# modelscope/FunCodec

Hardware: NVIDIA H100
Metric: codec frames/sec (encode+RVQ+decode) (higher is better)
Workload: dtype f32

## Files before the change

### funcodec_b200/csrc/rvq_tc.cu

```cuda
#include <climits>
#include "common.cuh"
#include "kernels.h"
#include "tc_sm90.cuh"

namespace fcb {

using namespace tc;

constexpr int RQ_M = 128;
constexpr int RQ_N = RVQ_TC_N;
constexpr int RQ_NB = 2;
constexpr int RQ_THREADS = 160;
constexpr float RQ_RESCORE_TOL = 4e-3f;

struct RqSmem {
    int a_slab;
    int off_b, off_cc, off_xx, off_idx, off_cand, off_bar, total;
};

__host__ __device__ inline RqSmem rq_layout(int D, int K) {
    RqSmem L;
    const int n_chunks = D / 32;
    L.a_slab = RQ_M * 128;
    L.off_b = 2 * n_chunks * L.a_slab;
    L.off_cc = L.off_b + RQ_NB * 2 * RQ_N * 128;
    L.off_xx = L.off_cc + K * 4;
    L.off_idx = L.off_xx + RQ_M * 4;
    L.off_cand = L.off_idx + RQ_M * 4;
    L.off_bar = (L.off_cand + 4 * RQ_M * 4 + 15) & ~15;
    L.total = L.off_bar + 8 * (2 * RQ_NB) + 16;
    return L;
}

__global__ void __launch_bounds__(RQ_THREADS, 1) rvq_tc_kernel(const RvqParams p) {
    extern __shared__ __align__(1024) uint8_t smem_raw[];
    const int tid = threadIdx.x, lane = tid & 31, warp = tid >> 5;
    const int D = p.D, K = p.K, T = p.T;
    const int n_chunks = D / 32;
    const int n_nt = K / RQ_N;
    const RqSmem L = rq_layout(D, K);
    const long long M = (long long)p.B * T;
    const long long row0 = (long long)blockIdx.x * RQ_M;

    uint8_t* smA = smem_raw;
    uint8_t* smB = smem_raw + L.off_b;
    float* cc_s = reinterpret_cast<float*>(smem_raw + L.off_cc);
    float* xx_s = reinterpret_cast<float*>(smem_raw + L.off_xx);
    int* idx_s = reinterpret_cast<int*>(smem_raw + L.off_idx);
    float* cv1_s = reinterpret_cast<float*>(smem_raw + L.off_cand);
    float* cv2_s = cv1_s + RQ_M;
    int* ci1_s = reinterpret_cast<int*>(cv2_s + RQ_M);
    int* ci2_s = ci1_s + RQ_M;
    uint64_t* bars = reinterpret_cast<uint64_t*>(smem_raw + L.off_bar);
    uint64_t* b_full = bars;
    uint64_t* b_empty = b_full + RQ_NB;

    if (tid == 0) {
        for (int i = 0; i < RQ_NB; ++i) { mbar_init(b_full + i, 1); mbar_init(b_empty + i, 1); }
        mbar_fence_init();
    }
    __syncthreads();
    const long long slab_bytes = 2LL * RQ_N * 128;

    if (warp < 4) {
        const int jchunk = tid & 7, rsub = tid >> 3;
        for (int ch = 0; ch < n_chunks; ++ch) {
            uint8_t* hi = smA + (2 * ch) * L.a_slab;
            uint8_t* lo = hi + L.a_slab;
            for (int r = rsub; r < RQ_M; r += 16) {
                const long long row = row0 + r;
                float4 v = make_float4(0.f, 0.f, 0.f, 0.f);
                const int d = ch * 32 + jchunk * 4;
                if (row < M) {
                    const int b = (int)(row / T), t = (int)(row - (long long)b * T);
                    v = __ldg(reinterpret_cast<const float4*>(p.in.x + (long long)b * p.in.clip_stride + (long long)(p.in.row_off + t) * D + d));
                    if (p.in.stats) {
                        const float mean = p.in.stats[2 * b], rstd = p.in.stats[2 * b + 1];
                        const float4 g4 = __ldg(reinterpret_cast<const float4*>(p.in.gamma + d));
                        const float4 b4 = __ldg(reinterpret_cast<const float4*>(p.in.beta + d));
                        float a;
                        a = rstd * g4.x; v.x = fmaf(v.x, a, b4.x - a * mean);
                        a = rstd * g4.y; v.y = fmaf(v.y, a, b4.y - a * mean);
                        a = rstd * g4.z; v.z = fmaf(v.z, a, b4.z - a * mean);
                        a = rstd * g4.w; v.w = fmaf(v.w, a, b4.w - a * mean);
                    }
                    if (p.enc_out) *reinterpret_cast<float4*>(p.enc_out + row * D + d) = v;
                }
                float4 h, l;
                split_tf32(v.x, h.x, l.x); split_tf32(v.y, h.y, l.y); split_tf32(v.z, h.z, l.z); split_tf32(v.w, h.w, l.w);
                const uint32_t o = (uint32_t)r * 128u + (uint32_t)((jchunk ^ (r & 7)) << 4);
                *reinterpret_cast<float4*>(hi + o) = h;
                *reinterpret_cast<float4*>(lo + o) = l;
            }
        }
        const int myrow = tid;
        const uint32_t a_base = smem_u32(smA), b_base = smem_u32(smB);
        long long it = 0;
        auto lex_lt = [](float va, int ia, float vb, int ib) { return va < vb || (va == vb && ia < ib); };
        for (int q = 0; q < p.n_q; ++q) {
            const float* E = p.embed + (long long)q * K * D;
            asm volatile("bar.sync 1, 128;" ::: "memory");
            for (int r = rsub; r < RQ_M; r += 16) {
                float s = 0.f;
                for (int d = jchunk; d < D; d += 8) {
                    const uint32_t o = (uint32_t)r * 128u + (uint32_t)((((d & 31) >> 2) ^ (r & 7)) << 4) + (uint32_t)((d & 3) << 2);
                    const uint8_t* hi = smA + (2 * (d >> 5)) * L.a_slab;
                    const float v = *reinterpret_cast<const float*>(hi + o) + *reinterpret_cast<const float*>(hi + L.a_slab + o);
                    s = fmaf(v, v, s);
                }
                s += __shfl_xor_sync(0xffffffffu, s, 1);
                s += __shfl_xor_sync(0xffffffffu, s, 2);
                s += __shfl_xor_sync(0xffffffffu, s, 4);
                if (jchunk == 0) xx_s[r] = s;
            }
            for (int c = tid; c < K; c += 128) cc_s[c] = __ldg(p.cnorm + (long long)q * K + c);
            fence_proxy_async_smem();
            asm volatile("bar.sync 1, 128;" ::: "memory");
            const float xx = xx_s[myrow];
            float xr[4], bv1[4], bv2[4];
            int bi1[4], bi2[4];
#pragma unroll
            for (int k = 0; k < 4; ++k) {
                xr[k] = xx_s[64 * (k >> 1) + 16 * warp + (lane >> 2) + 8 * (k & 1)];
                bv1[k] = 3.402823466e38f; bv2[k] = 3.402823466e38f;
                bi1[k] = INT_MAX; bi2[k] = INT_MAX;
            }
            for (int nt = 0; nt < n_nt; ++nt) {
                float acc0[RQ_N / 2], acc1[RQ_N / 2];
                int prev = -1;
                for (int ch = 0; ch < n_chunks; ++ch, ++it) {
                    const int bs = (int)(it % RQ_NB);
                    mbar_wait(b_full + bs, (uint32_t)((it / RQ_NB) & 1));
                    const uint32_t a_hi0 = a_base + (2 * ch) * L.a_slab, a_lo0 = a_hi0 + L.a_slab;
                    const uint32_t b_hi0 = b_base + bs * (uint32_t)slab_bytes, b_lo0 = b_hi0 + RQ_N * 128;
                    wgmma_fence();
#pragma unroll
                    for (int ks = 0; ks < 4; ++ks) {
                        const uint64_t db_hi = make_desc_k_sw128(b_hi0 + ks * 32), db_lo = make_desc_k_sw128(b_lo0 + ks * 32);
                        const uint32_t accum = (ch | ks) != 0;
                        wgmma_m64n128k8_tf32(acc0, make_desc_k_sw128(a_lo0 + ks * 32), db_hi, accum);
                        wgmma_m64n128k8_tf32(acc0, make_desc_k_sw128(a_hi0 + ks * 32), db_lo, 1);
                        wgmma_m64n128k8_tf32(acc0, make_desc_k_sw128(a_hi0 + ks * 32), db_hi, 1);
                        wgmma_m64n128k8_tf32(acc1, make_desc_k_sw128(a_lo0 + 8192 + ks * 32), db_hi, accum);
                        wgmma_m64n128k8_tf32(acc1, make_desc_k_sw128(a_hi0 + 8192 + ks * 32), db_lo, 1);
                        wgmma_m64n128k8_tf32(acc1, make_desc_k_sw128(a_hi0 + 8192 + ks * 32), db_hi, 1);
                    }
                    wgmma_commit();
                    wgmma_wait<1>();
                    if (prev >= 0 && tid == 0) mbar_arrive(b_empty + prev);
                    prev = bs;
                }
                wgmma_wait<0>();
                reg_fence(acc0);
                reg_fence(acc1);
                if (tid == 0) mbar_arrive(b_empty + prev);
                auto scan = [&](const float (&a)[RQ_N / 2], int h) {
#pragma unroll
                    for (int j = 0; j < RQ_N / 8; ++j)
#pragma unroll
                        for (int e = 0; e < 2; ++e) {
                            const int k = 2 * h + e;
#pragma unroll
                            for (int x = 0; x < 2; ++x) {
                                const int c = nt * RQ_N + 8 * j + 2 * (lane & 3) + x;
                                const float tv = __fadd_rn(__fsub_rn(xr[k], 2.0f * a[4 * j + 2 * e + x]), cc_s[c]);
                                if (tv < bv1[k]) { bv2[k] = bv1[k]; bi2[k] = bi1[k]; bv1[k] = tv; bi1[k] = c; }
                                else if (tv < bv2[k]) { bv2[k] = tv; bi2[k] = c; }
                            }
                        }
                };
                scan(acc0, 0);
                scan(acc1, 1);
            }
#pragma unroll
            for (int k = 0; k < 4; ++k) {
#pragma unroll
                for (int o = 1; o <= 2; o <<= 1) {
                    const float ov1 = __shfl_xor_sync(0xffffffffu, bv1[k], o), ov2 = __shfl_xor_sync(0xffffffffu, bv2[k], o);
                    const int oi1 = __shfl_xor_sync(0xffffffffu, bi1[k], o), oi2 = __shfl_xor_sync(0xffffffffu, bi2[k], o);
                    if (lex_lt(ov1, oi1, bv1[k], bi1[k])) {
                        if (lex_lt(ov2, oi2, bv1[k], bi1[k])) { bv2[k] = ov2; bi2[k] = oi2; }
                        else { bv2[k] = bv1[k]; bi2[k] = bi1[k]; }
                        bv1[k] = ov1; bi1[k] = oi1;
                    } else if (lex_lt(ov1, oi1, bv2[k], bi2[k])) {
                        bv2[k] = ov1; bi2[k] = oi1;
                    }
                }
                if ((lane & 3) == 0) {
                    const int rr = 64 * (k >> 1) + 16 * warp + (lane >> 2) + 8 * (k & 1);
                    cv1_s[rr] = bv1[k]; ci1_s[rr] = bi1[k] == INT_MAX ? 0 : bi1[k];
                    cv2_s[rr] = bv2[k]; ci2_s[rr] = bi2[k] == INT_MAX ? -1 : bi2[k];
                }
            }
            asm volatile("bar.sync 1, 128;" ::: "memory");
            const float v1 = cv1_s[myrow], v2 = cv2_s[myrow];
            const int i1 = ci1_s[myrow], i2 = ci2_s[myrow];
            int best = i1;
            if (row0 + myrow < M && v2 - v1 < RQ_RESCORE_TOL + 2e-5f * fabsf(v1) && i2 >= 0) {
                float d1 = 0.f, d2 = 0.f;
                const float* c1 = E + (long long)i1 * D;
                const float* c2 = E + (long long)i2 * D;
                for (int d = 0; d < D; ++d) {
                    const uint32_t o = (uint32_t)myrow * 128u + (uint32_t)((((d & 31) >> 2) ^ (myrow & 7)) << 4) + (uint32_t)((d & 3) << 2);
                    const uint8_t* hi = smA + (2 * (d >> 5)) * L.a_slab;
                    const float x = *reinterpret_cast<const float*>(hi + o) + *reinterpret_cast<const float*>(hi + L.a_slab + o);
                    d1 = fmaf(x, __ldg(c1 + d), d1);
                    d2 = fmaf(x, __ldg(c2 + d), d2);
                }
                const float t1 = __fadd_rn(__fsub_rn(xx, 2.0f * d1), cc_s[i1]);
                const float t2 = __fadd_rn(__fsub_rn(xx, 2.0f * d2), cc_s[i2]);
                if (t2 < t1 || (t2 == t1 && i2 < i1)) best = i2;
            }
            idx_s[myrow] = best;
            if (row0 + myrow < M) p.codes[(long long)q * M + row0 + myrow] = (long long)best;
            asm volatile("bar.sync 1, 128;" ::: "memory");
            {
                constexpr int MAXCH = 4;
                float4 cv[MAXCH], nv[MAXCH];
                auto load_c = [&](int r, float4 (&dst)[MAXCH]) {
#pragma unroll
                    for (int ch = 0; ch < MAXCH; ++ch) {
                        dst[ch] = make_float4(0.f, 0.f, 0.f, 0.f);
                        if (ch < n_chunks && row0 + r < M)
                            dst[ch] = __ldg(reinterpret_cast<const float4*>(E + (long long)idx_s[r] * D + ch * 32 + jchunk * 4));
                    }
                };
                load_c(rsub, cv);
                for (int r = rsub; r < RQ_M; r += 16) {
                    if (r + 16 < RQ_M) load_c(r + 16, nv);
                    const long long row = row0 + r;
                    if (row < M) {
                        const uint32_t o = (uint32_t)r * 128u + (uint32_t)((jchunk ^ (r & 7)) << 4);
#pragma unroll
                        for (int ch = 0; ch < MAXCH; ++ch) {
                            if (ch < n_chunks) {
                                uint8_t* hi = smA + (2 * ch) * L.a_slab;
                                uint8_t* lo = hi + L.a_slab;
                                const float4 h0 = *reinterpret_cast<const float4*>(hi + o);
                                const float4 l0 = *reinterpret_cast<const float4*>(lo + o);
                                const float4 c4 = cv[ch];
                                float4 x;
                                x.x = (h0.x + l0.x) - c4.x; x.y = (h0.y + l0.y) - c4.y; x.z = (h0.z + l0.z) - c4.z; x.w = (h0.w + l0.w) - c4.w;
                                float4 h, l;
                                split_tf32(x.x, h.x, l.x); split_tf32(x.y, h.y, l.y); split_tf32(x.z, h.z, l.z); split_tf32(x.w, h.w, l.w);
                                *reinterpret_cast<float4*>(hi + o) = h;
                                *reinterpret_cast<float4*>(lo + o) = l;
                                if (p.sub_quants) {
                                    const int b = (int)(row / T), t = (int)(row - (long long)b * T);
                                    const int d = ch * 32 + jchunk * 4;
                                    float* sq = p.sub_quants + (((long long)q * p.B + b) * D + d) * T + t;
                                    sq[0] = c4.x; sq[(long long)T] = c4.y; sq[2LL * T] = c4.z; sq[3LL * T] = c4.w;
                                }
                            }
                        }
                    }
#pragma unroll
                    for (int ch = 0; ch < MAXCH; ++ch) cv[ch] = nv[ch];
                }
            }
        }
    } else if (warp == 4) {
        if (lane == 0) {
            long long it = 0;
            for (int q = 0; q < p.n_q; ++q) {
                const uint8_t* qbase = reinterpret_cast<const uint8_t*>(p.embed_tc) + (long long)q * n_nt * n_chunks * slab_bytes;
                for (int nt = 0; nt < n_nt; ++nt)
                    for (int ch = 0; ch < n_chunks; ++ch, ++it) {
                        const int bs = (int)(it % RQ_NB);
                        mbar_wait_backoff(b_empty + bs, (uint32_t)((it / RQ_NB) & 1) ^ 1, 64);
                        mbar_arrive_expect_tx(b_full + bs, (uint32_t)slab_bytes);
                        bulk_g2s(smB + bs * slab_bytes, qbase + ((long long)nt * n_chunks + ch) * slab_bytes, (uint32_t)slab_bytes, b_full + bs);
                    }
            }
        }
    }
}

bool rvq_tc_supported(int D, int K) {
    return D % 32 == 0 && D >= 32 && D <= 128 && K % RQ_N == 0 && rq_layout(D, K).total <= 225 * 1024;
}

cudaError_t launch_rvq_tc(const RvqParams& p, cudaStream_t st) {
    if (!rvq_tc_supported(p.D, p.K) || !p.embed_tc) return cudaErrorInvalidValue;
    const RqSmem L = rq_layout(p.D, p.K);
    {
        cudaError_t e = ensure_dynamic_smem((const void*)rvq_tc_kernel, 225 * 1024);
        if (e != cudaSuccess) return e;
    }
    const long long M = (long long)p.B * p.T;
    rvq_tc_kernel<<<(unsigned)((M + RQ_M - 1) / RQ_M), RQ_THREADS, L.total, st>>>(p);
    return cudaGetLastError();
}

}
```

### funcodec_b200/csrc/tc_sm90.cuh

```cuda
#pragma once
#include <cuda_runtime.h>
#include <stdint.h>

namespace fcb {
namespace tc {

__device__ __forceinline__ uint32_t smem_u32(const void* p) { return (uint32_t)__cvta_generic_to_shared(p); }

__device__ __forceinline__ void mbar_init(uint64_t* bar, uint32_t count) {
    asm volatile("mbarrier.init.shared::cta.b64 [%0], %1;" ::"r"(smem_u32(bar)), "r"(count) : "memory");
}
__device__ __forceinline__ void mbar_fence_init() { asm volatile("fence.mbarrier_init.release.cluster;" ::: "memory"); }
__device__ __forceinline__ void mbar_arrive(uint64_t* bar) {
    asm volatile("{\n\t.reg .b64 st;\n\tmbarrier.arrive.shared::cta.b64 st, [%0];\n\t}" ::"r"(smem_u32(bar)) : "memory");
}
__device__ __forceinline__ void mbar_arrive_expect_tx(uint64_t* bar, uint32_t bytes) {
    asm volatile("{\n\t.reg .b64 st;\n\tmbarrier.arrive.expect_tx.shared::cta.b64 st, [%0], %1;\n\t}" ::"r"(smem_u32(bar)), "r"(bytes)
                 : "memory");
}
__device__ __forceinline__ void mbar_arrive_if(uint64_t* bar, bool pred) {
    asm volatile("{\n\t.reg .pred p;\n\t.reg .b64 st;\n\tsetp.ne.b32 p, %1, 0;\n\t@p mbarrier.arrive.shared::cta.b64 st, [%0];\n\t}" ::"r"(
                     smem_u32(bar)),
                 "r"((uint32_t)pred)
                 : "memory");
}
__device__ __forceinline__ bool mbar_try_wait(uint64_t* bar, uint32_t parity) {
    uint32_t ok;
    asm volatile(
        "{\n\t.reg .pred p;\n\t"
        "mbarrier.try_wait.parity.shared::cta.b64 p, [%1], %2;\n\t"
        "selp.u32 %0, 1, 0, p;\n\t}"
        : "=r"(ok)
        : "r"(smem_u32(bar)), "r"(parity)
        : "memory");
    return ok != 0;
}
__device__ __forceinline__ void mbar_wait(uint64_t* bar, uint32_t parity) {
    while (!mbar_try_wait(bar, parity)) { }
}
__device__ __forceinline__ void mbar_wait_backoff(uint64_t* bar, uint32_t parity, unsigned ns) {
    while (!mbar_try_wait(bar, parity)) { __nanosleep(ns); }
}

__device__ __forceinline__ void mbar_wait_cluster_backoff(uint64_t* bar, uint32_t parity, unsigned ns) {
    for (;;) {
        uint32_t ok;
        asm volatile(
            "{\n\t.reg .pred p;\n\t"
            "mbarrier.try_wait.parity.acquire.cluster.shared::cta.b64 p, [%1], %2;\n\t"
            "selp.u32 %0, 1, 0, p;\n\t}"
            : "=r"(ok)
            : "r"(smem_u32(bar)), "r"(parity)
            : "memory");
        if (ok) return;
        __nanosleep(ns);
    }
}

__device__ __forceinline__ void fence_proxy_async_smem() { asm volatile("fence.proxy.async.shared::cta;" ::: "memory"); }

__device__ __forceinline__ uint32_t cluster_ctarank() {
    uint32_t r;
    asm volatile("mov.u32 %0, %%cluster_ctarank;" : "=r"(r));
    return r;
}
__device__ __forceinline__ uint32_t mapa_shared(uint32_t smem_addr, uint32_t rank) {
    uint32_t r;
    asm volatile("mapa.shared::cluster.u32 %0, %1, %2;" : "=r"(r) : "r"(smem_addr), "r"(rank));
    return r;
}
__device__ __forceinline__ void mbar_arrive_remote_if(uint32_t remote_bar, bool pred) {
    asm volatile("{\n\t.reg .pred p;\n\tsetp.ne.b32 p, %1, 0;\n\t@p mbarrier.arrive.release.cluster.shared::cluster.b64 _, [%0];\n\t}" ::"r"(
                     remote_bar),
                 "r"((uint32_t)pred)
                 : "memory");
}
__device__ __forceinline__ void bulk_s2peer(uint32_t dst_remote, const void* src_smem, uint32_t bytes, uint32_t bar_remote) {
    asm volatile("cp.async.bulk.shared::cluster.shared::cta.mbarrier::complete_tx::bytes [%0], [%1], %2, [%3];" ::"r"(dst_remote),
                 "r"(smem_u32(src_smem)), "r"(bytes), "r"(bar_remote)
                 : "memory");
}
__device__ __forceinline__ void cluster_sync() {
    asm volatile("barrier.cluster.arrive.release;\n\tbarrier.cluster.wait.acquire;" ::: "memory");
}

__device__ __forceinline__ void bulk_g2s(void* dst_smem, const void* src_gmem, uint32_t bytes, uint64_t* bar) {
    asm volatile("cp.async.bulk.shared::cluster.global.mbarrier::complete_tx::bytes [%0], [%1], %2, [%3];" ::"r"(smem_u32(dst_smem)),
                 "l"(src_gmem), "r"(bytes), "r"(smem_u32(bar))
                 : "memory");
}

__device__ __forceinline__ void tma_load_4d(void* dst_smem, const void* tmap, int c0, int c1, int c2, int c3, uint64_t* bar) {
    asm volatile(
        "cp.async.bulk.tensor.4d.shared::cluster.global.tile.mbarrier::complete_tx::bytes [%0], [%1, {%3, %4, %5, %6}], [%2];" ::"r"(
            smem_u32(dst_smem)),
        "l"(tmap), "r"(smem_u32(bar)), "r"(c0), "r"(c1), "r"(c2), "r"(c3)
        : "memory");
}

__device__ __forceinline__ void tma_load_5d(void* dst_smem, const void* tmap, int c0, int c1, int c2, int c3, int c4, uint64_t* bar) {
    asm volatile(
        "cp.async.bulk.tensor.5d.shared::cluster.global.tile.mbarrier::complete_tx::bytes [%0], [%1, {%3, %4, %5, %6, %7}], [%2];" ::"r"(
            smem_u32(dst_smem)),
        "l"(tmap), "r"(smem_u32(bar)), "r"(c0), "r"(c1), "r"(c2), "r"(c3), "r"(c4)
        : "memory");
}

template <int R>
__device__ __forceinline__ void setmaxnreg_dec() { asm volatile("setmaxnreg.dec.sync.aligned.u32 %0;" ::"n"(R)); }
template <int R>
__device__ __forceinline__ void setmaxnreg_inc() { asm volatile("setmaxnreg.inc.sync.aligned.u32 %0;" ::"n"(R)); }

__device__ __forceinline__ void wgmma_fence() { asm volatile("wgmma.fence.sync.aligned;" ::: "memory"); }
__device__ __forceinline__ void wgmma_commit() { asm volatile("wgmma.commit_group.sync.aligned;" ::: "memory"); }
template <int N>
__device__ __forceinline__ void wgmma_wait() { asm volatile("wgmma.wait_group.sync.aligned %0;" ::"n"(N) : "memory"); }
template <int R>
__device__ __forceinline__ void reg_fence(float (&d)[R]) {
#pragma unroll
    for (int i = 0; i < R; ++i) asm volatile("" : "+f"(d[i])::"memory");
}

__device__ __forceinline__ void wgmma_m64n16k16_f16(float (&d)[8], uint64_t desc_a, uint64_t desc_b, uint32_t accumulate) {
    asm volatile(
        "{\n\t.reg .pred p;\n\t"
        "setp.ne.b32 p, %10, 0;\n\t"
        "wgmma.mma_async.sync.aligned.m64n16k16.f32.f16.f16 "
        "{%0, %1, %2, %3, %4, %5, %6, %7}, %8, %9, p, 1, 1, 0, 0;\n\t}"
        : "+f"(d[0]), "+f"(d[1]), "+f"(d[2]), "+f"(d[3]), "+f"(d[4]), "+f"(d[5]), "+f"(d[6]), "+f"(d[7])
        : "l"(desc_a), "l"(desc_b), "r"(accumulate));
}

__device__ __forceinline__ void wgmma_m64n32k16_f16(float (&d)[16], uint64_t desc_a, uint64_t desc_b, uint32_t accumulate) {
    asm volatile(
        "{\n\t.reg .pred p;\n\t"
        "setp.ne.b32 p, %18, 0;\n\t"
        "wgmma.mma_async.sync.aligned.m64n32k16.f32.f16.f16 "
        "{%0, %1, %2, %3, %4, %5, %6, %7, %8, %9, %10, %11, %12, %13, %14, %15}, %16, %17, p, 1, 1, 0, 0;\n\t}"
        : "+f"(d[0]), "+f"(d[1]), "+f"(d[2]), "+f"(d[3]), "+f"(d[4]), "+f"(d[5]), "+f"(d[6]), "+f"(d[7]), "+f"(d[8]), "+f"(d[9]), "+f"(d[10]), "+f"(d[11]), "+f"(d[12]), "+f"(d[13]), "+f"(d[14]), "+f"(d[15])
        : "l"(desc_a), "l"(desc_b), "r"(accumulate));
}

__device__ __forceinline__ void wgmma_m64n64k16_f16(float (&d)[32], uint64_t desc_a, uint64_t desc_b, uint32_t accumulate) {
    asm volatile(
        "{\n\t.reg .pred p;\n\t"
        "setp.ne.b32 p, %34, 0;\n\t"
        "wgmma.mma_async.sync.aligned.m64n64k16.f32.f16.f16 "
        "{%0, %1, %2, %3, %4, %5, %6, %7, %8, %9, %10, %11, %12, %13, %14, %15, %16, %17, %18, %19, %20, %21, %22, %23, %24, %25, %26, %27, %28, %29, %30, %31}, %32, %33, p, 1, 1, 0, 0;\n\t}"
        : "+f"(d[0]), "+f"(d[1]), "+f"(d[2]), "+f"(d[3]), "+f"(d[4]), "+f"(d[5]), "+f"(d[6]), "+f"(d[7]), "+f"(d[8]), "+f"(d[9]), "+f"(d[10]), "+f"(d[11]), "+f"(d[12]), "+f"(d[13]), "+f"(d[14]), "+f"(d[15]), "+f"(d[16]), "+f"(d[17]), "+f"(d[18]), "+f"(d[19]), "+f"(d[20]), "+f"(d[21]), "+f"(d[22]), "+f"(d[23]), "+f"(d[24]), "+f"(d[25]), "+f"(d[26]), "+f"(d[27]), "+f"(d[28]), "+f"(d[29]), "+f"(d[30]), "+f"(d[31])
        : "l"(desc_a), "l"(desc_b), "r"(accumulate));
}

__device__ __forceinline__ void wgmma_m64n128k16_f16(float (&d)[64], uint64_t desc_a, uint64_t desc_b, uint32_t accumulate) {
    asm volatile(
        "{\n\t.reg .pred p;\n\t"
        "setp.ne.b32 p, %66, 0;\n\t"
        "wgmma.mma_async.sync.aligned.m64n128k16.f32.f16.f16 "
        "{%0, %1, %2, %3, %4, %5, %6, %7, %8, %9, %10, %11, %12, %13, %14, %15, %16, %17, %18, %19, %20, %21, %22, %23, %24, %25, %26, %27, %28, %29, %30, %31, %32, %33, %34, %35, %36, %37, %38, %39, %40, %41, %42, %43, %44, %45, %46, %47, %48, %49, %50, %51, %52, %53, %54, %55, %56, %57, %58, %59, %60, %61, %62, %63}, %64, %65, p, 1, 1, 0, 0;\n\t}"
        : "+f"(d[0]), "+f"(d[1]), "+f"(d[2]), "+f"(d[3]), "+f"(d[4]), "+f"(d[5]), "+f"(d[6]), "+f"(d[7]), "+f"(d[8]), "+f"(d[9]), "+f"(d[10]), "+f"(d[11]), "+f"(d[12]), "+f"(d[13]), "+f"(d[14]), "+f"(d[15]), "+f"(d[16]), "+f"(d[17]), "+f"(d[18]), "+f"(d[19]), "+f"(d[20]), "+f"(d[21]), "+f"(d[22]), "+f"(d[23]), "+f"(d[24]), "+f"(d[25]), "+f"(d[26]), "+f"(d[27]), "+f"(d[28]), "+f"(d[29]), "+f"(d[30]), "+f"(d[31]), "+f"(d[32]), "+f"(d[33]), "+f"(d[34]), "+f"(d[35]), "+f"(d[36]), "+f"(d[37]), "+f"(d[38]), "+f"(d[39]), "+f"(d[40]), "+f"(d[41]), "+f"(d[42]), "+f"(d[43]), "+f"(d[44]), "+f"(d[45]), "+f"(d[46]), "+f"(d[47]), "+f"(d[48]), "+f"(d[49]), "+f"(d[50]), "+f"(d[51]), "+f"(d[52]), "+f"(d[53]), "+f"(d[54]), "+f"(d[55]), "+f"(d[56]), "+f"(d[57]), "+f"(d[58]), "+f"(d[59]), "+f"(d[60]), "+f"(d[61]), "+f"(d[62]), "+f"(d[63])
        : "l"(desc_a), "l"(desc_b), "r"(accumulate));
}

__device__ __forceinline__ void wgmma_m64n128k8_tf32(float (&d)[64], uint64_t desc_a, uint64_t desc_b, uint32_t accumulate) {
    asm volatile(
        "{\n\t.reg .pred p;\n\t"
        "setp.ne.b32 p, %66, 0;\n\t"
        "wgmma.mma_async.sync.aligned.m64n128k8.f32.tf32.tf32 "
        "{%0, %1, %2, %3, %4, %5, %6, %7, %8, %9, %10, %11, %12, %13, %14, %15, %16, %17, %18, %19, %20, %21, %22, %23, %24, %25, %26, %27, %28, %29, %30, %31, %32, %33, %34, %35, %36, %37, %38, %39, %40, %41, %42, %43, %44, %45, %46, %47, %48, %49, %50, %51, %52, %53, %54, %55, %56, %57, %58, %59, %60, %61, %62, %63}, %64, %65, p, 1, 1;\n\t}"
        : "+f"(d[0]), "+f"(d[1]), "+f"(d[2]), "+f"(d[3]), "+f"(d[4]), "+f"(d[5]), "+f"(d[6]), "+f"(d[7]), "+f"(d[8]), "+f"(d[9]), "+f"(d[10]), "+f"(d[11]), "+f"(d[12]), "+f"(d[13]), "+f"(d[14]), "+f"(d[15]), "+f"(d[16]), "+f"(d[17]), "+f"(d[18]), "+f"(d[19]), "+f"(d[20]), "+f"(d[21]), "+f"(d[22]), "+f"(d[23]), "+f"(d[24]), "+f"(d[25]), "+f"(d[26]), "+f"(d[27]), "+f"(d[28]), "+f"(d[29]), "+f"(d[30]), "+f"(d[31]), "+f"(d[32]), "+f"(d[33]), "+f"(d[34]), "+f"(d[35]), "+f"(d[36]), "+f"(d[37]), "+f"(d[38]), "+f"(d[39]), "+f"(d[40]), "+f"(d[41]), "+f"(d[42]), "+f"(d[43]), "+f"(d[44]), "+f"(d[45]), "+f"(d[46]), "+f"(d[47]), "+f"(d[48]), "+f"(d[49]), "+f"(d[50]), "+f"(d[51]), "+f"(d[52]), "+f"(d[53]), "+f"(d[54]), "+f"(d[55]), "+f"(d[56]), "+f"(d[57]), "+f"(d[58]), "+f"(d[59]), "+f"(d[60]), "+f"(d[61]), "+f"(d[62]), "+f"(d[63])
        : "l"(desc_a), "l"(desc_b), "r"(accumulate));
}

template <int N> struct WgmmaF16;
template <> struct WgmmaF16<16> { static __device__ __forceinline__ void mma(float (&d)[8], uint64_t a, uint64_t b, uint32_t acc) { wgmma_m64n16k16_f16(d, a, b, acc); } };
template <> struct WgmmaF16<32> { static __device__ __forceinline__ void mma(float (&d)[16], uint64_t a, uint64_t b, uint32_t acc) { wgmma_m64n32k16_f16(d, a, b, acc); } };
template <> struct WgmmaF16<64> { static __device__ __forceinline__ void mma(float (&d)[32], uint64_t a, uint64_t b, uint32_t acc) { wgmma_m64n64k16_f16(d, a, b, acc); } };
template <> struct WgmmaF16<128> { static __device__ __forceinline__ void mma(float (&d)[64], uint64_t a, uint64_t b, uint32_t acc) { wgmma_m64n128k16_f16(d, a, b, acc); } };

__device__ __forceinline__ uint64_t make_desc_k_sw128(uint32_t addr) {
    uint64_t d = 0;
    d |= (uint64_t)((addr & 0x3FFFFu) >> 4);
    d |= (uint64_t)1 << 16;
    d |= (uint64_t)(1024 >> 4) << 32;
    d |= (uint64_t)1 << 62;
    return d;
}
__device__ __forceinline__ uint32_t sw128_offset(uint32_t row, uint32_t col) {
    return row * 128u + ((((col >> 2) ^ (row & 7u)) << 4) | ((col & 3u) << 2));
}

__device__ __forceinline__ void split_f16x2(float x0, float x1, uint32_t& hi, uint32_t& lo) {
    asm("cvt.rn.satfinite.f16x2.f32 %0, %1, %2;" : "=r"(hi) : "f"(x1), "f"(x0));
    float f0, f1;
    asm("{\n\t.reg .b16 l, h;\n\tmov.b32 {l, h}, %2;\n\tcvt.f32.f16 %0, l;\n\tcvt.f32.f16 %1, h;\n\t}" : "=f"(f0), "=f"(f1) : "r"(hi));
    asm("cvt.rn.satfinite.f16x2.f32 %0, %1, %2;" : "=r"(lo) : "f"(x1 - f1), "f"(x0 - f0));
}
__device__ __forceinline__ float exp2f_approx(float x) {
    float y;
    asm("ex2.approx.ftz.f32 %0, %1;" : "=f"(y) : "f"(x));
    return y;
}

__device__ __forceinline__ void split_tf32(float x, float& hi, float& lo) {
    uint32_t u = __float_as_uint(x);
    u = (u + 0x1000u) & 0xFFFFE000u;
    hi = __uint_as_float(u);
    lo = x - hi;
}

}
}
```

Baseline: 145,500.

## Split RVQ codebook search across thread-block cluster ranks with DSMEM candidate exchange

Each 128-row tile is now processed by a cluster of up to 4 CTAs, with each CTA scanning a disjoint slice of codebook N-tiles. Per-row top-2 candidates are pushed to peer CTAs over distributed shared memory using bulk copies and an mbarrier, then merged locally. Output writes are partitioned by row range among the ranks. The goal is more SM parallelism when there are too few row tiles to fill the GPU. The cost is redundant residual and update work in every CTA plus cluster synchronisation overhead. Cluster mode is used only when the tile count fits the occupancy limit.

Measured after the change: 150,300 (median of 6 runs). 1.03x the previous value.

```diff
diff --git a/funcodec_b200/csrc/rvq_tc.cu b/funcodec_b200/csrc/rvq_tc.cu
--- a/funcodec_b200/csrc/rvq_tc.cu
+++ b/funcodec_b200/csrc/rvq_tc.cu
@@ -11,6 +11,8 @@
 constexpr int RQ_N = RVQ_TC_N;
 constexpr int RQ_NB = 2;
 constexpr int RQ_THREADS = 160;
+constexpr int RQ_MAX_RANKS = 4;
+constexpr int RQ_CAND_BYTES = 4 * RQ_M * 4;
 constexpr float RQ_RESCORE_TOL = 4e-3f;
 
 struct RqSmem {
@@ -18,7 +20,7 @@
     int off_b, off_cc, off_xx, off_idx, off_cand, off_bar, total;
 };
 
-__host__ __device__ inline RqSmem rq_layout(int D, int K) {
+__host__ __device__ inline RqSmem rq_layout(int D, int K, int s) {
     RqSmem L;
     const int n_chunks = D / 32;
     L.a_slab = RQ_M * 128;
@@ -27,8 +29,8 @@
     L.off_xx = L.off_cc + K * 4;
     L.off_idx = L.off_xx + RQ_M * 4;
     L.off_cand = L.off_idx + RQ_M * 4;
-    L.off_bar = (L.off_cand + 4 * RQ_M * 4 + 15) & ~15;
-    L.total = L.off_bar + 8 * (2 * RQ_NB) + 16;
+    L.off_bar = (L.off_cand + (s > 1 ? 2 : 1) * s * RQ_CAND_BYTES + 15) & ~15;
+    L.total = L.off_bar + 8 * (2 * RQ_NB + 2) + 16;
     return L;
 }
 
@@ -38,28 +40,30 @@
     const int D = p.D, K = p.K, T = p.T;
     const int n_chunks = D / 32;
     const int n_nt = K / RQ_N;
-    const RqSmem L = rq_layout(D, K);
+    const int s = (int)cluster_nctarank(), rank = s > 1 ? (int)cluster_ctarank() : 0;
+    const int n_loc = n_nt / s, nt0 = rank * n_loc;
+    const int own_lo = rank * (RQ_M / s), own_hi = own_lo + RQ_M / s;
+    const RqSmem L = rq_layout(D, K, s);
     const long long M = (long long)p.B * T;
-    const long long row0 = (long long)blockIdx.x * RQ_M;
+    const long long row0 = (long long)(blockIdx.x / s) * RQ_M;
 
     uint8_t* smA = smem_raw;
     uint8_t* smB = smem_raw + L.off_b;
     float* cc_s = reinterpret_cast<float*>(smem_raw + L.off_cc);
     float* xx_s = reinterpret_cast<float*>(smem_raw + L.off_xx);
     int* idx_s = reinterpret_cast<int*>(smem_raw + L.off_idx);
-    float* cv1_s = reinterpret_cast<float*>(smem_raw + L.off_cand);
-    float* cv2_s = cv1_s + RQ_M;
-    int* ci1_s = reinterpret_cast<int*>(cv2_s + RQ_M);
-    int* ci2_s = ci1_s + RQ_M;
+    float* cand_s = reinterpret_cast<float*>(smem_raw + L.off_cand);
     uint64_t* bars = reinterpret_cast<uint64_t*>(smem_raw + L.off_bar);
     uint64_t* b_full = bars;
     uint64_t* b_empty = b_full + RQ_NB;
+    uint64_t* c_full = b_empty + RQ_NB;
 
     if (tid == 0) {
         for (int i = 0; i < RQ_NB; ++i) { mbar_init(b_full + i, 1); mbar_init(b_empty + i, 1); }
+        for (int i = 0; i < 2; ++i) mbar_init(c_full + i, 1);
         mbar_fence_init();
     }
-    __syncthreads();
+    if (s > 1) cluster_sync(); else __syncthreads();
     const long long slab_bytes = 2LL * RQ_N * 128;
 
     if (warp < 4) {
@@ -84,7 +88,7 @@
                         a = rstd * g4.z; v.z = fmaf(v.z, a, b4.z - a * mean);
                         a = rstd * g4.w; v.w = fmaf(v.w, a, b4.w - a * mean);
                     }
-                    if (p.enc_out) *reinterpret_cast<float4*>(p.enc_out + row * D + d) = v;
+                    if (p.enc_out && r >= own_lo && r < own_hi) *reinterpret_cast<float4*>(p.enc_out + row * D + d) = v;
                 }
                 float4 h, l;
                 split_tf32(v.x, h.x, l.x); split_tf32(v.y, h.y, l.y); split_tf32(v.z, h.z, l.z); split_tf32(v.w, h.w, l.w);
@@ -94,24 +98,37 @@
             }
         }
         const int myrow = tid;
+        const bool own_row = myrow >= own_lo && myrow < own_hi;
         const uint32_t a_base = smem_u32(smA), b_base = smem_u32(smB);
         long long it = 0;
         auto lex_lt = [](float va, int ia, float vb, int ib) { return va < vb || (va == vb && ia < ib); };
+        auto merge2 = [&](float& v1, int& i1, float& v2, int& i2, float ov1, int oi1, float ov2, int oi2) {
+            if (lex_lt(ov1, oi1, v1, i1)) {
+                if (lex_lt(ov2, oi2, v1, i1)) { v2 = ov2; i2 = oi2; }
+                else { v2 = v1; i2 = i1; }
+                v1 = ov1; i1 = oi1;
+            } else if (lex_lt(ov1, oi1, v2, i2)) {
+                v2 = ov1; i2 = oi1;
+            }
+        };
         for (int q = 0; q < p.n_q; ++q) {
             const float* E = p.embed + (long long)q * K * D;
+            const int cb = s > 1 ? (q & 1) : 0;
+            float* cand_cb = cand_s + cb * s * (4 * RQ_M);
             asm volatile("bar.sync 1, 128;" ::: "memory");
+            if (s > 1 && tid == 0) mbar_arrive_expect_tx(c_full + cb, (uint32_t)((s - 1) * RQ_CAND_BYTES));
             for (int r = rsub; r < RQ_M; r += 16) {
-                float s = 0.f;
+                float sum = 0.f;
                 for (int d = jchunk; d < D; d += 8) {
                     const uint32_t o = (uint32_t)r * 128u + (uint32_t)((((d & 31) >> 2) ^ (r & 7)) << 4) + (uint32_t)((d & 3) << 2);
                     const uint8_t* hi = smA + (2 * (d >> 5)) * L.a_slab;
                     const float v = *reinterpret_cast<const float*>(hi + o) + *reinterpret_cast<const float*>(hi + L.a_slab + o);
-                    s = fmaf(v, v, s);
-                }
-                s += __shfl_xor_sync(0xffffffffu, s, 1);
-                s += __shfl_xor_sync(0xffffffffu, s, 2);
-                s += __shfl_xor_sync(0xffffffffu, s, 4);
-                if (jchunk == 0) xx_s[r] = s;
+                    sum = fmaf(v, v, sum);
+                }
+                sum += __shfl_xor_sync(0xffffffffu, sum, 1);
+                sum += __shfl_xor_sync(0xffffffffu, sum, 2);
+                sum += __shfl_xor_sync(0xffffffffu, sum, 4);
+                if (jchunk == 0) xx_s[r] = sum;
             }
             for (int c = tid; c < K; c += 128) cc_s[c] = __ldg(p.cnorm + (long long)q * K + c);
             fence_proxy_async_smem();
@@ -125,7 +142,7 @@
                 bv1[k] = 3.402823466e38f; bv2[k] = 3.402823466e38f;
                 bi1[k] = INT_MAX; bi2[k] = INT_MAX;
             }
-            for (int nt = 0; nt < n_nt; ++nt) {
+            for (int nt = nt0; nt < nt0 + n_loc; ++nt) {
                 float acc0[RQ_N / 2], acc1[RQ_N / 2];
                 int prev = -1;
                 for (int ch = 0; ch < n_chunks; ++ch, ++it) {
@@ -172,29 +189,43 @@
                 scan(acc0, 0);
                 scan(acc1, 1);
             }
+            float* own = cand_cb + rank * (4 * RQ_M);
 #pragma unroll
             for (int k = 0; k < 4; ++k) {
 #pragma unroll
                 for (int o = 1; o <= 2; o <<= 1) {
                     const float ov1 = __shfl_xor_sync(0xffffffffu, bv1[k], o), ov2 = __shfl_xor_sync(0xffffffffu, bv2[k], o);
                     const int oi1 = __shfl_xor_sync(0xffffffffu, bi1[k], o), oi2 = __shfl_xor_sync(0xffffffffu, bi2[k], o);
-                    if (lex_lt(ov1, oi1, bv1[k], bi1[k])) {
-                        if (lex_lt(ov2, oi2, bv1[k], bi1[k])) { bv2[k] = ov2; bi2[k] = oi2; }
-                        else { bv2[k] = bv1[k]; bi2[k] = bi1[k]; }
-                        bv1[k] = ov1; bi1[k] = oi1;
-                    } else if (lex_lt(ov1, oi1, bv2[k], bi2[k])) {
-                        bv2[k] = ov1; bi2[k] = oi1;
-                    }
+                    merge2(bv1[k], bi1[k], bv2[k], bi2[k], ov1, oi1, ov2, oi2);
                 }
                 if ((lane & 3) == 0) {
                     const int rr = 64 * (k >> 1) + 16 * warp + (lane >> 2) + 8 * (k & 1);
-                    cv1_s[rr] = bv1[k]; ci1_s[rr] = bi1[k] == INT_MAX ? 0 : bi1[k];
-                    cv2_s[rr] = bv2[k]; ci2_s[rr] = bi2[k] == INT_MAX ? -1 : bi2[k];
-                }
-            }
-            asm volatile("bar.sync 1, 128;" ::: "memory");
-            const float v1 = cv1_s[myrow], v2 = cv2_s[myrow];
-            const int i1 = ci1_s[myrow], i2 = ci2_s[myrow];
+                    own[rr] = bv1[k]; reinterpret_cast<int*>(own)[RQ_M + rr] = bi1[k];
+                    own[2 * RQ_M + rr] = bv2[k]; reinterpret_cast<int*>(own)[3 * RQ_M + rr] = bi2[k];
+                }
+            }
+            if (s > 1) {
+                fence_proxy_async_smem();
+                asm volatile("bar.sync 1, 128;" ::: "memory");
+                if (tid == 0) {
+                    for (int j = 1; j < s; ++j) {
+                        const uint32_t peer = (uint32_t)((rank + j) % s);
+                        bulk_s2peer(mapa_shared(smem_u32(own), peer), own, (uint32_t)RQ_CAND_BYTES, mapa_shared(smem_u32(c_full + cb), peer));
+                    }
+                }
+                mbar_wait_cluster_backoff(c_full + cb, (uint32_t)((q >> 1) & 1), 32);
+            } else {
+                asm volatile("bar.sync 1, 128;" ::: "memory");
+            }
+            float v1 = 3.402823466e38f, v2 = 3.402823466e38f;
+            int i1 = INT_MAX, i2 = INT_MAX;
+            for (int r = 0; r < s; ++r) {
+                const float* l = cand_cb + r * (4 * RQ_M);
+                merge2(v1, i1, v2, i2, l[myrow], reinterpret_cast<const int*>(l)[RQ_M + myrow], l[2 * RQ_M + myrow],
+                       reinterpret_cast<const int*>(l)[3 * RQ_M + myrow]);
+            }
+            if (i1 == INT_MAX) i1 = 0;
+            if (i2 == INT_MAX) i2 = -1;
             int best = i1;
             if (row0 + myrow < M && v2 - v1 < RQ_RESCORE_TOL + 2e-5f * fabsf(v1) && i2 >= 0) {
                 float d1 = 0.f, d2 = 0.f;
@@ -212,7 +243,7 @@
                 if (t2 < t1 || (t2 == t1 && i2 < i1)) best = i2;
             }
             idx_s[myrow] = best;
-            if (row0 + myrow < M) p.codes[(long long)q * M + row0 + myrow] = (long long)best;
+            if (row0 + myrow < M && own_row) p.codes[(long long)q * M + row0 + myrow] = (long long)best;
             asm volatile("bar.sync 1, 128;" ::: "memory");
             {
                 constexpr int MAXCH = 4;
@@ -245,7 +276,7 @@
                                 split_tf32(x.x, h.x, l.x); split_tf32(x.y, h.y, l.y); split_tf32(x.z, h.z, l.z); split_tf32(x.w, h.w, l.w);
                                 *reinterpret_cast<float4*>(hi + o) = h;
                                 *reinterpret_cast<float4*>(lo + o) = l;
-                                if (p.sub_quants) {
+                                if (p.sub_quants && r >= own_lo && r < own_hi) {
                                     const int b = (int)(row / T), t = (int)(row - (long long)b * T);
                                     const int d = ch * 32 + jchunk * 4;
                                     float* sq = p.sub_quants + (((long long)q * p.B + b) * D + d) * T + t;
@@ -264,7 +295,7 @@
             long long it = 0;
             for (int q = 0; q < p.n_q; ++q) {
                 const uint8_t* qbase = reinterpret_cast<const uint8_t*>(p.embed_tc) + (long long)q * n_nt * n_chunks * slab_bytes;
-                for (int nt = 0; nt < n_nt; ++nt)
+                for (int nt = nt0; nt < nt0 + n_loc; ++nt)
                     for (int ch = 0; ch < n_chunks; ++ch, ++it) {
                         const int bs = (int)(it % RQ_NB);
                         mbar_wait_backoff(b_empty + bs, (uint32_t)((it / RQ_NB) & 1) ^ 1, 64);
@@ -274,21 +305,52 @@
             }
         }
     }
+    if (s > 1) cluster_sync();
 }
 
 bool rvq_tc_supported(int D, int K) {
-    return D % 32 == 0 && D >= 32 && D <= 128 && K % RQ_N == 0 && rq_layout(D, K).total <= 225 * 1024;
-}
+    return D % 32 == 0 && D >= 32 && D <= 128 && K % RQ_N == 0 && rq_layout(D, K, 1).total <= 225 * 1024;
+}
+
+constexpr int RQ_DEVICES = 64;
+static int g_rq_max_clusters[RQ_DEVICES][2] = {};
 
 cudaError_t launch_rvq_tc(const RvqParams& p, cudaStream_t st) {
     if (!rvq_tc_supported(p.D, p.K) || !p.embed_tc) return cudaErrorInvalidValue;
-    const RqSmem L = rq_layout(p.D, p.K);
     {
         cudaError_t e = ensure_dynamic_smem((const void*)rvq_tc_kernel, 225 * 1024);
         if (e != cudaSuccess) return e;
     }
     const long long M = (long long)p.B * p.T;
-    rvq_tc_kernel<<<(unsigned)((M + RQ_M - 1) / RQ_M), RQ_THREADS, L.total, st>>>(p);
+    const long long tiles = (M + RQ_M - 1) / RQ_M;
+    for (int s = RQ_MAX_RANKS; s > 1; s >>= 1) {
+        if ((p.K / RQ_N) % s != 0 || rq_layout(p.D, p.K, s).total > 225 * 1024) continue;
+        cudaLaunchAttribute attr[1];
+        attr[0].id = cudaLaunchAttributeClusterDimension;
+        attr[0].val.clusterDim.x = (unsigned)s; attr[0].val.clusterDim.y = 1; attr[0].val.clusterDim.z = 1;
+        cudaLaunchConfig_t cfg = {};
+        cfg.blockDim = dim3(RQ_THREADS);
+        cfg.stream = st;
+        cfg.attrs = attr;
+        cfg.numAttrs = 1;
+        int dev = 0;
+        cudaError_t e = cudaGetDevice(&dev);
+        if (e != cudaSuccess) return e;
+        int max_clusters = dev < RQ_DEVICES ? g_rq_max_clusters[dev][s / 2 - 1] : 0;
+        if (max_clusters == 0) {
+            cfg.gridDim = dim3((unsigned)s);
+            cfg.dynamicSmemBytes = 225 * 1024;
+            e = cudaOccupancyMaxActiveClusters(&max_clusters, rvq_tc_kernel, &cfg);
+            if (e != cudaSuccess) return e;
+            if (max_clusters < 1) max_clusters = -1;
+            if (dev < RQ_DEVICES) g_rq_max_clusters[dev][s / 2 - 1] = max_clusters;
+        }
+        if (tiles > max_clusters) continue;
+        cfg.gridDim = dim3((unsigned)(tiles * s));
+        cfg.dynamicSmemBytes = rq_layout(p.D, p.K, s).total;
+        return cudaLaunchKernelEx(&cfg, rvq_tc_kernel, p);
+    }
+    rvq_tc_kernel<<<(unsigned)tiles, RQ_THREADS, rq_layout(p.D, p.K, 1).total, st>>>(p);
     return cudaGetLastError();
 }
 
diff --git a/funcodec_b200/csrc/tc_sm90.cuh b/funcodec_b200/csrc/tc_sm90.cuh
--- a/funcodec_b200/csrc/tc_sm90.cuh
+++ b/funcodec_b200/csrc/tc_sm90.cuh
@@ -64,6 +64,11 @@
     asm volatile("mov.u32 %0, %%cluster_ctarank;" : "=r"(r));
     return r;
 }
+__device__ __forceinline__ uint32_t cluster_nctarank() {
+    uint32_t r;
+    asm volatile("mov.u32 %0, %%cluster_nctarank;" : "=r"(r));
+    return r;
+}
 __device__ __forceinline__ uint32_t mapa_shared(uint32_t smem_addr, uint32_t rank) {
     uint32_t r;
     asm volatile("mapa.shared::cluster.u32 %0, %1, %2;" : "=r"(r) : "r"(smem_addr), "r"(rank));
```
